# BlockstreamResearch/secp256k1-zkp

Measured on AMD Instinct MI355X. Metric: 64-bit Borromean rangeproof verifies/sec, higher is better.
Workload: dtype u32 limbs (9x29-bit), 32x32->64 integer MAC

## Files before the change

### __graft_entry__.py

```python
import os
import subprocess
import sys

ROOT = os.path.dirname(os.path.abspath(__file__))
CSRC = os.path.join(ROOT, "secp256k1_zkp_amd", "csrc")
HIPCC = os.environ.get("HIPCC", "/opt/rocm/bin/hipcc")
HIP_FLAGS = ["--offload-arch=gfx950", "-O3", "-std=c++17", "-shared", "-fPIC", "-Wno-unused-value"]


def _run(cmd, cwd=None):
    print("+", " ".join(cmd), flush=True)
    subprocess.check_call(cmd, cwd=cwd)


def _stale(target, sources):
    if not os.path.exists(target):
        return True
    t = os.path.getmtime(target)
    return any(os.path.getmtime(s) > t for s in sources if os.path.exists(s))


def build(force=False):
    hdrs = [os.path.join(CSRC, f) for f in os.listdir(CSRC) if f.endswith((".h", ".hip"))] + [os.path.join(ROOT, "include", "secp256k1_zkp_amd.h")]
    sys.path.insert(0, ROOT)
    from secp256k1_zkp_amd import build_lib
    build_lib.build(force=force)
    prims_src = os.path.join(ROOT, "tests", "gpu_prims", "prims.hip")
    prims = os.path.join(ROOT, "tests", "gpu_prims", "libs2k_gpuprims.so")
    if force or _stale(prims, hdrs + [prims_src]):
        _run([HIPCC] + HIP_FLAGS + ["-o", prims, prims_src])
    winv_src = os.path.join(ROOT, "tests", "wave_inverse", "waveinv_test.hip")
    winv = os.path.join(ROOT, "tests", "wave_inverse", "libs2k_waveinv_test.so")
    if force or _stale(winv, hdrs + [winv_src]):
        _run([HIPCC] + HIP_FLAGS + ["-o", winv, winv_src])
    wlanes_src = os.path.join(ROOT, "tests", "wave_inverse", "waveinv_lanes_test.hip")
    wlanes = os.path.join(ROOT, "tests", "wave_inverse", "libs2k_waveinv_lanes_test.so")
    if force or _stale(wlanes, hdrs + [wlanes_src]):
        _run([HIPCC] + HIP_FLAGS + ["-o", wlanes, wlanes_src])
    emu_src = os.path.join(ROOT, "tests", "host_emul", "hostemu.cpp")
    emu = os.path.join(ROOT, "tests", "host_emul", "libs2k_hostemu.so")
    if force or _stale(emu, hdrs + [emu_src]):
        _run(["g++", "-O2", "-std=c++17", "-fPIC", "-shared", "-o", emu, emu_src])
    ecdsa_emu_src = os.path.join(ROOT, "tests", "host_emul", "ecdsa_emu.cpp")
    ecdsa_emu = os.path.join(ROOT, "tests", "host_emul", "libs2k_ecdsa_emu.so")
    if force or _stale(ecdsa_emu, hdrs + [emu_src, ecdsa_emu_src]):
        _run(["g++", "-O2", "-std=c++17", "-fPIC", "-shared", "-o", ecdsa_emu, ecdsa_emu_src])
    wl_emu_src = os.path.join(ROOT, "tests", "host_emul", "whitelist_emu.cpp")
    wl_emu = os.path.join(ROOT, "tests", "host_emul", "libs2k_whitelist_emu.so")
    if force or _stale(wl_emu, hdrs + [emu_src, wl_emu_src]):
        _run(["g++", "-O2", "-std=c++17", "-fPIC", "-shared", "-o", wl_emu, wl_emu_src])
    tw_emu_src = os.path.join(ROOT, "tests", "host_emul", "tweak_emu.cpp")
    tw_emu = os.path.join(ROOT, "tests", "host_emul", "libs2k_tweak_emu.so")
    if force or _stale(tw_emu, hdrs + [emu_src, tw_emu_src]):
        _run(["g++", "-O2", "-std=c++17", "-fPIC", "-shared", "-o", tw_emu, tw_emu_src])
    gen_emu_src = os.path.join(ROOT, "tests", "host_emul", "generator_emu.cpp")
    gen_emu = os.path.join(ROOT, "tests", "host_emul", "libs2k_generator_emu.so")
    if force or _stale(gen_emu, hdrs + [emu_src, gen_emu_src]):
        _run(["g++", "-O2", "-std=c++17", "-fPIC", "-shared", "-o", gen_emu, gen_emu_src])
    ad_emu_src = os.path.join(ROOT, "tests", "host_emul", "adaptor_emu.cpp")
    ad_emu = os.path.join(ROOT, "tests", "host_emul", "libs2k_adaptor_emu.so")
    if force or _stale(ad_emu, hdrs + [emu_src, ad_emu_src]):
        _run(["g++", "-O2", "-std=c++17", "-fPIC", "-shared", "-o", ad_emu, ad_emu_src])
    if os.path.exists(os.path.join(ROOT, "oracle", "zkp_oracle.c")):
        _run(["make", "-s", "-C", os.path.join(ROOT, "oracle"), "oracle"])
    if os.path.isdir(os.environ.get("S2K_REFERENCE", "/root/reference")):
        _run(["make", "-s", "-C", os.path.join(ROOT, "oracle"), "ref", "hooked", "benches", "routed"])
    sys.path.insert(0, ROOT)
    import secp256k1_zkp_amd
    from secp256k1_zkp_amd import _native
    _native.load()


def smoke():
    sys.path.insert(0, ROOT)
    from tests import smoke_impl
    smoke_impl.run()


if __name__ == "__main__":
    build(force="--force" in sys.argv)
    if "--smoke" in sys.argv:
        smoke()
```

### secp256k1_zkp_amd/csrc/ecmult.h

```cpp
#pragma once
#include "group.h"
#include "scalar.h"

#ifndef S2K_GTAB_BITS
#define S2K_GTAB_BITS 26
#endif
#define S2K_GTAB_MAX_BITS 26
#define S2K_GTAB_ENTRY_WORDS 16
#define S2K_GTAB_SWORDS 9
#define S2K_GTAB_MAX_WINDOWS 32
struct gtab_geom { u32 D, W; };
S2K_HD u32 gtab_windows_for(u32 D) { return (256u + D - 1u) / D; }
S2K_HD u32 gtab_top_bits_for(u32 D) { return 256u - D * (gtab_windows_for(D) - 1u); }
S2K_HD int gtab_bits_ok(u32 D) { return D >= 8u && D <= S2K_GTAB_MAX_BITS && gtab_top_bits_for(D) >= 1u && gtab_top_bits_for(D) < D - 1u; }
S2K_HD size_t gtab_slot(u32 D, u32 w, u32 v) { return ((size_t)w << (D - 1u)) + (size_t)v; }
S2K_HD size_t gtab_slots_for(u32 D) { return gtab_slot(D, gtab_windows_for(D), 0) + 1; }
S2K_HD size_t gtab_words_for(u32 D) { return gtab_slots_for(D) * S2K_GTAB_ENTRY_WORDS; }
S2K_HD gtab_geom gtab_geometry(const u32* tab) { gtab_geom g; g.D = tab[0]; g.W = tab[1]; return g; }
S2K_HD void gtab_write_header(u32* tab, u32 D) {
    const u32 W = gtab_windows_for(D);
    tab[0] = D; tab[1] = W;
    for (int i = 0; i < S2K_GTAB_SWORDS; i++) {
        u32 k = 0;
        for (u32 w = 0; w + 1 < W; w++) { const u32 bit = D - 1u + D * w; if ((bit >> 5) == (u32)i) k |= 1u << (bit & 31u); }
        tab[2 + i] = k;
    }
    for (int i = 2 + S2K_GTAB_SWORDS; i < S2K_GTAB_ENTRY_WORDS; i++) tab[i] = 0;
}

S2K_HD void gtab_load(ge& r, const u32* gtab, u32 window, u32 v) {
    const u32* p = gtab + gtab_slot(gtab[0], window, v) * S2K_GTAB_ENTRY_WORDS;
    u32 w[16];
#pragma unroll
    for (int i = 0; i < 16; i++) w[i] = p[i];
    fe_from_words(r.x, w); fe_from_words(r.y, w + 8);
}
S2K_HD void gtab_recode(u32 out[S2K_GTAB_SWORDS], const u32 s[8], const u32* tab) {
    u64 cy = 0;
#pragma unroll
    for (int i = 0; i < S2K_GTAB_SWORDS; i++) {
        cy += (u64)(i < 8 ? s[i] : 0u) + tab[2 + i];
        out[i] = (u32)cy; cy >>= 32;
    }
}
S2K_HD int gtab_locate(const u32*& addr, int& neg, const u32* tab, const gtab_geom& G, int g, u32 lo, u32 hi) {
    const u32 b = (u32)g * G.D;
    const u64 pair = (u64)lo | ((u64)hi << 32);
    const u32 t = (u32)(pair >> (b & 31u)) & ((1u << G.D) - 1u);
    u32 v;
    if ((u32)g + 1u < G.W) { const int d = (int)t - (int)(1u << (G.D - 1u)); neg = d < 0; v = (u32)(d < 0 ? -d : d); }
    else { neg = 0; v = t; }
    if (!v) return 0;
    addr = tab + gtab_slot(G.D, (u32)g, v) * S2K_GTAB_ENTRY_WORDS;
    return 1;
}

#ifndef S2K_PTAB_TWINS
#define S2K_PTAB_TWINS 0
#endif
#define S2K_PTAB_ENTRIES 8
#define S2K_PTAB_ENTRY_WORDS 32
#define S2K_PTAB_TABLE_WORDS (S2K_PTAB_ENTRIES * S2K_PTAB_ENTRY_WORDS)
#define S2K_PTAB_ZISO (2 * S2K_PTAB_TABLE_WORDS)
#define S2K_PTAB_NG (S2K_PTAB_ZISO + 9)
#define S2K_PTAB_WORDS (2 * S2K_PTAB_TABLE_WORDS + 32)

#if defined(__HIP_DEVICE_COMPILE__)
#define S2K_LD_NT(p) __builtin_nontemporal_load(p)
#define S2K_ST_NT(v, p) __builtin_nontemporal_store((v), (p))
#else
#define S2K_LD_NT(p) (*(p))
#define S2K_ST_NT(v, p) (*(p) = (v))
#endif
#ifndef S2K_NT_PARK
#define S2K_NT_PARK 1
#endif
#ifndef S2K_XYZZ_TABLE_PART
#define S2K_XYZZ_TABLE_PART 1
#endif
#ifndef S2K_NT_GTAB_SPLIT
#define S2K_NT_GTAB_SPLIT 0
#endif
#ifndef S2K_NT_GTAB
#define S2K_NT_GTAB 1
#endif
template <int WS = 1>
S2K_HD void ptab_store_raw(u32* e, const fe& x, const fe& y, const fe& third) {
#pragma unroll
    for (int i = 0; i < 9; i++) {
        if (S2K_NT_PARK && WS > 1) { S2K_ST_NT(x.n[i], &e[i * WS]); S2K_ST_NT(y.n[i], &e[(9 + i) * WS]); S2K_ST_NT(third.n[i], &e[(18 + i) * WS]); }
        else { e[i * WS] = x.n[i]; e[(9 + i) * WS] = y.n[i]; e[(18 + i) * WS] = third.n[i]; }
    }
}
template <int N, int WS = 1, int ES = S2K_PTAB_ENTRY_WORDS>
S2K_HD void ptab_build_raw_n(fe& ziso, u32* tab, const gej& A) {
    fe x = A.x, y = A.y; fe_norm_weak(x); fe_norm_weak(y);
    fe zc, s, t, l, nx, s2, qx, qy, w, px, py;
    fe_mul_sqr(zc, y, A.z, s, y);
    fe_neg(nx, x, 1);
    fe_mul_sqr(t, nx, s, l, x);
    fe_mul_int(l, 3); fe_half(l); fe_norm_weak(l);
    fe_sqr2(qx, l, s2, s);
    fe_add(qx, t); fe_add(qx, t); fe_norm_weak(qx);
    fe_add2(w, qx, t);
    fe_mul(qy, l, w); fe_add(qy, s2); fe_neg(qy, qy, 2); fe_norm_weak(qy);
    fe_neg(px, t, 1); py = s2;
    { fe one; fe_set_int(one, 1); ptab_store_raw<WS>(tab, px, py, one); }
    for (int i = 1; i < N; i++) {
        fe dx, dy, c, d, w1, w2, e, a1, x3, y3, tmp;
        fe_neg(dx, px, 4); fe_add(dx, qx); fe_norm_weak(dx);
        fe_neg(dy, py, 3); fe_add(dy, qy); fe_norm_weak(dy);
        fe_sqr2(c, dx, d, dy);
        fe_mul2(w1, qx, c, w2, px, c);
        fe_neg(e, w2, 1); fe_add(e, w1);
        fe_add2(tmp, w1, w2); fe_neg(tmp, tmp, 2);
        fe_add2(x3, d, tmp);
        fe_neg(tmp, x3, 4); fe_add(tmp, w1);
        fe_mul2(a1, qy, e, y3, dy, tmp);
        fe_neg(tmp, a1, 1); fe_add(y3, tmp);
        fe_mul(zc, zc, dx);
        ptab_store_raw<WS>(tab + i * ES, x3, y3, dx);
        px = x3; py = y3; qx = w1; qy = a1;
    }
    ziso = zc;
}
S2K_HD void ptab_build_raw(fe& ziso, u32* tab, const gej& A) { ptab_build_raw_n<S2K_PTAB_ENTRIES>(ziso, tab, A); }
template <int N, int WS = 1, int ES = S2K_PTAB_ENTRY_WORDS>
S2K_HD void ptab_rescale_n(u32* tab, u32* fin, int fin_stride, const fe* zs0) {
    fe zs; if (zs0) zs = *zs0; else fe_set_int(zs, 1);
    u32 nraw[27];
    fe x, y, h;
#pragma unroll
    for (int k = 0; k < 27; k++) nraw[k] = (S2K_NT_PARK && WS > 1) ? S2K_LD_NT(&tab[(N - 1) * ES + k * WS]) : tab[(N - 1) * ES + k * WS];
#pragma unroll
    for (int k = 0; k < 9; k++) { x.n[k] = nraw[k]; y.n[k] = nraw[9 + k]; h.n[k] = nraw[18 + k]; }
    for (int i = N - 1; i >= 0; i--) {
        const u32* er = tab + i * ES;
        u32* e = fin + i * fin_stride;
        if (i > 0) {
#pragma unroll
            for (int k = 0; k < 27; k++) nraw[k] = (S2K_NT_PARK && WS > 1) ? S2K_LD_NT(&er[k * WS - ES]) : er[k * WS - ES];
        }
        if (zs0 || i != N - 1) {
            fe zs2, zs3; fe_sqr(zs2, zs); fe_mul(zs3, zs2, zs);
            fe_mul(x, x, zs2); fe_mul(y, y, zs3);
        }
        fe_normalize(x); fe_normalize(y);
        u32 wx[8], wy[8];
        fe_to_words(wx, x); fe_to_words(wy, y);
#pragma unroll
        for (int k = 0; k < 8; k++) { e[k] = wx[k]; e[8 + k] = wy[k]; }
#if S2K_PTAB_TWINS
        {
            fe beta, bx; fe_set_beta(beta);
            fe_mul(bx, x, beta); fe_normalize(bx);
            u32 wb[8]; fe_to_words(wb, bx);
#pragma unroll
            for (int k = 0; k < 8; k++) { e[16 + k] = wb[k]; e[24 + k] = wy[k]; }
        }
#endif
        fe_mul(zs, zs, h);
        if (i > 0) {
#pragma unroll
            for (int k = 0; k < 27; k++) S2K_CHAIN(nraw[k]);
#pragma unroll
            for (int k = 0; k < 9; k++) { x.n[k] = nraw[k]; y.n[k] = nraw[9 + k]; h.n[k] = nraw[18 + k]; }
        }
    }
}
S2K_HD void ptab_rescale(u32* tab, const fe* zs0) { ptab_rescale_n<S2K_PTAB_ENTRIES>(tab, tab, S2K_PTAB_ENTRY_WORDS, zs0); }
S2K_HD void ptab_build(fe& ziso, u32* ptab, const gej& A) {
    ptab_build_raw(ziso, ptab, A);
    ptab_rescale(ptab, nullptr);
}
S2K_HD void ptab_load_ziso(fe& zi, const u32* ptab) {
#pragma unroll
    for (int i = 0; i < 9; i++) zi.n[i] = ptab[S2K_PTAB_ZISO + i];
}

#if defined(__HIP_DEVICE_COMPILE__)
#define S2K_WAVE_ANY(p) (__any(p))
#define S2K_WAVE_ALL(p) (__all(p))
#define S2K_UNIFORM(x) (__builtin_amdgcn_readfirstlane(x))
#else
#define S2K_WAVE_ANY(p) (p)
#define S2K_WAVE_ALL(p) (p)
#define S2K_UNIFORM(x) (x)
#endif

#define S2K_DIG_WORDS 18
#if defined(__HIP_DEVICE_COMPILE__)
typedef __attribute__((address_space(3))) u32* s2k_lds_ptr;
#define S2K_DIG_STRIDE 256
#define S2K_LANE_DIG(shared_array) ((s2k_lds_ptr)(shared_array) + threadIdx.x)
#else
typedef u32* s2k_lds_ptr;
#define S2K_DIG_STRIDE 1
#define S2K_LANE_DIG(array) (array)
#endif
struct lane_mem { u32* ptab; s2k_lds_ptr dig; };

struct digit_reg { u32 w[5]; };
S2K_HD void digit_reg_init(digit_reg& r, const u32 k[5]) {
    r.w[4] = (k[4] << 31) | (k[3] >> 1);
    r.w[3] = (k[3] << 31) | (k[2] >> 1);
    r.w[2] = (k[2] << 31) | (k[1] >> 1);
    r.w[1] = (k[1] << 31) | (k[0] >> 1);
    r.w[0] = (k[0] << 31);
}
S2K_HD u32 digit_reg_pop(digit_reg& r) {
    const u32 v = r.w[4] >> 28;
#pragma unroll
    for (int i = 4; i > 0; i--) r.w[i] = (r.w[i] << 4) | (r.w[i - 1] >> 28);
    r.w[0] <<= 4;
    return v;
}

#define S2K_ADDS_P 66
#define S2K_ADD_G0 S2K_ADDS_P
#define S2K_ADDS_MAX (S2K_ADD_G0 + S2K_GTAB_MAX_WINDOWS)

S2K_HD void ecmult_lane(gej& R, const gej& A, const scalar& na, const scalar& ng, int has_ng, const u32* gtab, const lane_mem& lm) {
    u32* const ptab = lm.ptab; const s2k_lds_ptr dig = lm.dig;
    S2K_PROF_DECL;
    const int p_active = (!A.inf) & (!sc_is_zero(na));
    const int g_active = has_ng & (!sc_is_zero(ng));
    int hneg0, hneg1;
    fe ziso;
    {
        half_scalar h0, h1;
        sc_split_lambda_odd(h0, h1, na);
        hneg0 = h0.neg; hneg1 = h1.neg;
        {
            digit_reg dr0, dr1; digit_reg_init(dr0, h0.w); digit_reg_init(dr1, h1.w);
            u32 dw[9];
#pragma unroll
            for (int i = 0; i < 9; i++) dw[i] = 0;
#pragma unroll
            for (int i = 2; i < S2K_ADDS_P; i++) { const u32 v = (i & 1) ? digit_reg_pop(dr1) : digit_reg_pop(dr0); dw[i >> 3] |= v << ((i & 7) * 4); }
#pragma unroll
            for (int i = 0; i < 9; i++) dig[i * S2K_DIG_STRIDE] = dw[i];
        }
        S2K_PROF_MARK(1);
        if (S2K_WAVE_ANY(p_active)) {
            ptab_build(ziso, ptab, A);
#pragma unroll
            for (int i = 0; i < 9; i++) ptab[S2K_PTAB_ZISO + i] = ziso.n[i];
        }
    }
    const gtab_geom GG = gtab_geometry(gtab);
    {
        u32 ngr[S2K_GTAB_SWORDS]; gtab_recode(ngr, ng.d, gtab);
#pragma unroll
        for (int i = 0; i < S2K_GTAB_SWORDS; i++) dig[(9 + i) * S2K_DIG_STRIDE] = ngr[i];
    }

    S2K_PROF_MARK(2);
    int a = p_active ? 0 : S2K_ADD_G0;
    int zfixed = !p_active;
    int dbl_left = 0, pending = 0;
    const int a_end = g_active ? S2K_ADD_G0 + (int)GG.W : S2K_ADD_G0;
    auto op_locate = [&](const u32*& addr, int& valid, int& neg, int& lam, int idx) {
        addr = ptab; valid = 0; neg = 0; lam = 0;
        if (idx < S2K_ADD_G0) {
            const int h = idx & 1;
            const int hn = h ? hneg1 : hneg0;
            u32 v = 8u; int flip = hn; valid = 1;
            if (idx >= 2 && idx < S2K_ADDS_P) v = (dig[(idx >> 3) * S2K_DIG_STRIDE] >> ((idx & 7) * 4)) & 15u;
            neg = (v < 8u) ^ flip;
            const u32 e = (v < 8u) ? (7u - v) : (v - 8u);
            addr = ptab + e * S2K_PTAB_ENTRY_WORDS + ((h && S2K_PTAB_TWINS) ? 16 : 0); lam = h && !S2K_PTAB_TWINS;
        } else if (idx < a_end) {
            const int g = idx - S2K_ADD_G0, w = (int)(((u32)g * GG.D) >> 5);
            valid = gtab_locate(addr, neg, gtab, GG, g, dig[(9 + w) * S2K_DIG_STRIDE], w + 1 < S2K_GTAB_SWORDS ? dig[(10 + w) * S2K_DIG_STRIDE] : 0u);
        }
    };
    auto op_decode = [&](ge& o, const u32 raw[16], int neg, int lam) {
        fe y, yn;
        fe_from_words(o.x, raw); fe_from_words(y, raw + 8);
        if (S2K_WAVE_ANY(lam)) {
            fe beta, bx; fe_set_beta(beta); fe_mul(bx, o.x, beta);
            fe_select(o.x, bx, o.x, lam);
        }
        fe_neg(yn, y, 1);
        fe_select(o.y, yn, y, neg);
    };
    const u32* nxt_addr; int nxt_valid, nxt_neg, nxt_lam;
    u32 raw[16];
    ge cur; int cur_valid;
    op_locate(nxt_addr, nxt_valid, nxt_neg, nxt_lam, a);
#pragma unroll
    for (int k = 0; k < 16; k++) raw[k] = nxt_addr[k];
    op_decode(cur, raw, nxt_neg, nxt_lam); cur_valid = nxt_valid;
    gej_set_infinity(R);
    if (p_active) {
        gej_set_ge(R, cur);
        a = 1;
        op_locate(nxt_addr, nxt_valid, nxt_neg, nxt_lam, a);
#pragma unroll
        for (int k = 0; k < 16; k++) raw[k] = nxt_addr[k];
        op_decode(cur, raw, nxt_neg, nxt_lam); cur_valid = nxt_valid;
    }
    op_locate(nxt_addr, nxt_valid, nxt_neg, nxt_lam, a + 1);
#ifndef S2K_NO_FAST_PATH
    if (S2K_WAVE_ALL(p_active) && (S2K_WAVE_ALL(g_active) || !S2K_WAVE_ANY(g_active))) {
        int au = 1;
        while (au < a_end) {
            if (au >= 2 && au < S2K_ADDS_P && !(au & 1)) {
#pragma unroll 1
                for (int k = 0; k < 4; k++) gej_double_lean(R, R);
                S2K_PROF_MARK(6);
            }
            if (au == S2K_ADD_G0) { fe zi; ptab_load_ziso(zi, ptab); fe_mul(R.z, R.z, zi); zfixed = 1; }
#pragma unroll
            for (int k = 0; k < 16; k++) raw[k] = nxt_addr[k];
            gej t; const int same_x = gej_add_ge_lean(t, R, cur);
            if (S2K_WAVE_ANY(same_x & cur_valid)) break;
            if (au < S2K_ADDS_P) R = t;
            else if (cur_valid) R = t;
            au++;
            op_decode(cur, raw, nxt_neg, nxt_lam); cur_valid = nxt_valid;
            op_locate(nxt_addr, nxt_valid, nxt_neg, nxt_lam, au + 1);
        }
        if (au == S2K_ADD_G0 && !zfixed) { fe zi; ptab_load_ziso(zi, ptab); fe_mul(R.z, R.z, zi); zfixed = 1; }
        a = au;
    }
#endif
    int done = !(a < a_end) & zfixed;
    while (S2K_WAVE_ANY(!done)) {
        int do_dbl = 0, do_add = 0;
        if (!done) {
            if (pending) { do_dbl = 1; pending = 0; }
            else if (dbl_left > 0) { do_dbl = !R.inf; dbl_left--; }
            else do_add = 1;
        }
        if (S2K_WAVE_ANY(do_dbl)) {
            gej t; gej_double(t, R);
            if (do_dbl) R = t;
        }
        if (S2K_WAVE_ANY(do_add)) {
#pragma unroll
            for (int k = 0; k < 16; k++) raw[k] = nxt_addr[k];
            gej t; const int f = gej_add_ge(t, R, cur);
            ge nx; op_decode(nx, raw, nxt_neg, nxt_lam);
            if (do_add) {
                if (cur_valid) { R = t; pending = (f == GEJ_ADD_NEEDS_DOUBLE); }
                a++;
                cur = nx; cur_valid = nxt_valid;
                dbl_left = (a >= 2 && a < S2K_ADDS_P && !(a & 1)) ? 4 : 0;
                op_locate(nxt_addr, nxt_valid, nxt_neg, nxt_lam, a + 1);
            }
        }
        const int fix = (!done) & (!zfixed) & (a == S2K_ADD_G0) & (!pending);
        if (S2K_WAVE_ANY(fix)) {
            fe zi;
#pragma unroll
            for (int i = 0; i < 9; i++) zi.n[i] = ptab[S2K_PTAB_ZISO + i];
            fe z; fe_mul(z, R.z, zi);
            if (fix) { R.z = z; zfixed = 1; }
        }
        if ((a >= a_end) & (!pending) & zfixed) done = 1;
    }
    S2K_PROF_MARK(3);
}


#define S2K_SPLIT_ADDS_P 68
struct piece65 { u32 w[3]; int neg; };
S2K_HD void sc_split_pieces(piece65 out[4], const half_scalar& h0, const half_scalar& h1) {
    for (int hf = 0; hf < 2; hf++) {
        const half_scalar& h = hf ? h1 : h0;
        u32 lo[3] = {h.w[0], h.w[1], 0u};
        u32 hi[3] = {h.w[2], h.w[3], h.w[4]};
        int lo_neg = h.neg;
        if (!(hi[0] & 1u)) {
            u32 c = 1u;
            for (int i = 0; i < 3; i++) { const u32 t = hi[i] + c; c = (t < c); hi[i] = t; }
            const u64 l = (u64)lo[0] | ((u64)lo[1] << 32);
            const u64 m = 0ull - l;
            lo[0] = (u32)m; lo[1] = (u32)(m >> 32); lo[2] = 0u;
            lo_neg = !h.neg;
        }
        for (int i = 0; i < 3; i++) { out[hf].w[i] = lo[i]; out[2 + hf].w[i] = hi[i]; }
        out[hf].neg = lo_neg; out[2 + hf].neg = h.neg;
    }
}
S2K_HD int ecmult_lane_split(gej& R, const gej& A, const gej& T, const scalar& na, const scalar& ng, int has_ng, const u32* gtab, const lane_mem& lm) {
    u32* const ptab = lm.ptab; const s2k_lds_ptr dig = lm.dig;
    const int p_active = (!A.inf) & (!T.inf) & (!sc_is_zero(na));
    const int g_active = has_ng & (!sc_is_zero(ng));
    if (!(S2K_WAVE_ALL(p_active) && (S2K_WAVE_ALL(g_active) || !S2K_WAVE_ANY(g_active)))) return 0;
    u32 sneg = 0;
    S2K_PROF_DECL;
    {
        half_scalar h0, h1; sc_split_lambda_odd(h0, h1, na);
        piece65 pc[4]; sc_split_pieces(pc, h0, h1);
        u32 dw[8];
#pragma unroll
        for (int i = 0; i < 8; i++) dw[i] = 0;
#pragma unroll
        for (int st = 0; st < 4; st++) {
            sneg |= (u32)pc[st].neg << st;
#pragma unroll
            for (int pos = 0; pos < 16; pos++) {
                const int i = 15 - pos, bit = 4 * i + 1, word = bit >> 5, sh = bit & 31;
                const u64 pair = (u64)pc[st].w[word] | ((u64)(word + 1 < 3 ? pc[st].w[word + 1] : 0u) << 32);
                const u32 v = (u32)(pair >> sh) & 15u;
                const int nib = pos * 4 + st;
                dw[nib >> 3] |= v << ((nib & 7) * 4);
            }
        }
#pragma unroll
        for (int i = 0; i < 8; i++) dig[i * S2K_DIG_STRIDE] = dw[i];
        {
            u32 ngr[S2K_GTAB_SWORDS]; gtab_recode(ngr, ng.d, gtab);
#pragma unroll
            for (int i = 0; i < S2K_GTAB_SWORDS; i++) dig[(8 + i) * S2K_DIG_STRIDE] = ngr[i];
        }
        fe za, zt, ziso;
        S2K_PROF_MARK(1);
        ptab_build_raw(za, ptab, A);
        ptab_build_raw(zt, ptab + S2K_PTAB_TABLE_WORDS, T);
        S2K_PROF_MARK(8);
        ptab_rescale(ptab, &zt);
        ptab_rescale(ptab + S2K_PTAB_TABLE_WORDS, &za);
        S2K_PROF_MARK(9);
        fe_mul(ziso, za, zt);
#pragma unroll
        for (int i = 0; i < 9; i++) ptab[S2K_PTAB_ZISO + i] = ziso.n[i];
    }
    const gtab_geom GG = gtab_geometry(gtab);
    const int a_g0 = S2K_SPLIT_ADDS_P;
    const int a_end = g_active ? a_g0 + (int)GG.W : a_g0;
    auto op_locate = [&](const u32*& addr, int& valid, int& neg, int& lam, int idx) {
        addr = ptab; valid = 0; neg = 0; lam = 0;
        if (idx < a_g0) {
            const int st = idx & 3;
            u32 v = 8u;
            if (idx >= 4) { const int nib = idx - 4; v = (dig[(nib >> 3) * S2K_DIG_STRIDE] >> ((nib & 7) * 4)) & 15u; }
            valid = 1;
            neg = (v < 8u) ^ (int)((sneg >> st) & 1u);
            const u32 e = (v < 8u) ? (7u - v) : (v - 8u);
            addr = ptab + (st >> 1) * S2K_PTAB_TABLE_WORDS + e * S2K_PTAB_ENTRY_WORDS + (((st & 1) && S2K_PTAB_TWINS) ? 16 : 0); lam = (st & 1) && !S2K_PTAB_TWINS;
        } else if (idx < a_end) {
            const int g = idx - a_g0, w = (int)(((u32)g * GG.D) >> 5);
            valid = gtab_locate(addr, neg, gtab, GG, g, dig[(8 + w) * S2K_DIG_STRIDE], w + 1 < S2K_GTAB_SWORDS ? dig[(9 + w) * S2K_DIG_STRIDE] : 0u);
        }
    };
    auto op_decode = [&](ge& o, const u32 raw[16], int neg, int lam) {
        fe y, yn;
        fe_from_words(o.x, raw); fe_from_words(y, raw + 8);
        if (lam) { fe beta; fe_set_beta(beta); fe_mul(o.x, o.x, beta); }
        fe_neg(yn, y, 1);
        fe_select(o.y, yn, y, neg);
    };
    const u32* nxt_addr; int nxt_valid, nxt_neg, nxt_lam;
    u32 raw[16];
    ge cur; int cur_valid;
    op_locate(nxt_addr, nxt_valid, nxt_neg, nxt_lam, 0);
#pragma unroll
    for (int k = 0; k < 16; k++) raw[k] = nxt_addr[k];
    op_decode(cur, raw, nxt_neg, 0);
    op_locate(nxt_addr, nxt_valid, nxt_neg, nxt_lam, 1);
    int au = 0;
    while (au < a_g0) {
        if (au >= 4 && !(au & 3)) {
#pragma unroll 1
            for (int k = 0; k < 4; k++) gej_double_lean(R, R);
            S2K_PROF_MARK(6);
        }
#pragma unroll
        for (int k = 0; k < 16; k++) raw[k] = nxt_addr[k];
        if (au == 0) gej_set_ge(R, cur);
        else { const int same_x = gej_add_ge_lean(R, R, cur); if (S2K_WAVE_ANY(same_x)) return 0; }
        op_decode(cur, raw, nxt_neg, !S2K_PTAB_TWINS);
        op_locate(nxt_addr, nxt_valid, nxt_neg, nxt_lam, au + 2);
#pragma unroll
        for (int k = 0; k < 16; k++) raw[k] = nxt_addr[k];
        { const int same_x = gej_add_ge_lean(R, R, cur); if (S2K_WAVE_ANY(same_x)) return 0; }
        au += 2;
        op_decode(cur, raw, nxt_neg, 0); cur_valid = nxt_valid;
        op_locate(nxt_addr, nxt_valid, nxt_neg, nxt_lam, au + 1);
    }
    { fe zi; ptab_load_ziso(zi, ptab); fe_mul(R.z, R.z, zi); }
#if S2K_XYZZ_TABLE_PART
    gez acc4; acc4.inf = 0; acc4.x = R.x; acc4.y = R.y;
    fe_sqr(acc4.zz, R.z); fe_mul(acc4.zzz, acc4.zz, R.z);
#endif
    while (au < a_end) {
#if S2K_NT_GTAB_SPLIT && defined(__HIP_DEVICE_COMPILE__)
        {
            typedef unsigned int s2k_u32x4 __attribute__((ext_vector_type(4)));
            const s2k_u32x4* q = (const s2k_u32x4*)nxt_addr;
#pragma unroll
            for (int k = 0; k < 4; k++) { const s2k_u32x4 v = __builtin_nontemporal_load(q + k); raw[4 * k] = v.x; raw[4 * k + 1] = v.y; raw[4 * k + 2] = v.z; raw[4 * k + 3] = v.w; }
        }
#else
#pragma unroll
        for (int k = 0; k < 16; k++) raw[k] = nxt_addr[k];
#endif
#if S2K_XYZZ_TABLE_PART
        {
            gez t = acc4; gez_add_ge_lean(t, cur);
            if (S2K_WAVE_ALL(cur_valid)) acc4 = t;
            else { fe_cmov(acc4.x, t.x, cur_valid); fe_cmov(acc4.y, t.y, cur_valid); fe_cmov(acc4.zz, t.zz, cur_valid); fe_cmov(acc4.zzz, t.zzz, cur_valid); }
        }
#else
        gej t; const int same_x = gej_add_ge_lean(t, R, cur);
        if (S2K_WAVE_ANY(same_x & cur_valid)) return 0;
        if (cur_valid) R = t;
#endif
        au++;
        op_decode(cur, raw, nxt_neg, nxt_lam); cur_valid = nxt_valid;
        op_locate(nxt_addr, nxt_valid, nxt_neg, nxt_lam, au + 1);
    }
#if S2K_XYZZ_TABLE_PART
    if (S2K_WAVE_ANY(fe_normalizes_to_zero(acc4.zz))) return 0;
    gej_set_gez(R, acc4);
#endif
    S2K_PROF_MARK(10);
#ifdef S2K_ON_SPLIT_DONE
    S2K_ON_SPLIT_DONE();
#endif
    return 1;
}


#define S2K_RING_W 5
#define S2K_RING_ENTRIES 16
#define S2K_RING_DIGITS 13
#define S2K_RING_ADDS_P (4 * S2K_RING_DIGITS)
#define S2K_RING_DIG_WORDS 27
#define S2K_RTAB_TABLE_WORDS (S2K_RING_ENTRIES * 16)
#define S2K_RTAB_ZISO (2 * S2K_RTAB_TABLE_WORDS)
#define S2K_RTAB_WORDS (S2K_RTAB_ZISO + 16)
#if defined(__HIP_DEVICE_COMPILE__)
#define S2K_RAW_WS 64
#else
#define S2K_RAW_WS 1
#endif
#define S2K_RAW_ES (27 * S2K_RAW_WS)
#define S2K_RRAW_WAVE_WORDS (2 * S2K_RING_ENTRIES * 27 * 64)

S2K_HD void ecmult_ring_tables(u32* rtab, u32* raw, const gej& C, const gej& T) {
    fe za, zt, ziso;
    u32* const raw_t = raw + S2K_RING_ENTRIES * S2K_RAW_ES;
    ptab_build_raw_n<S2K_RING_ENTRIES, S2K_RAW_WS, S2K_RAW_ES>(za, raw, C);
    ptab_build_raw_n<S2K_RING_ENTRIES, S2K_RAW_WS, S2K_RAW_ES>(zt, raw_t, T);
    ptab_rescale_n<S2K_RING_ENTRIES, S2K_RAW_WS, S2K_RAW_ES>(raw, rtab, 16, &zt);
    ptab_rescale_n<S2K_RING_ENTRIES, S2K_RAW_WS, S2K_RAW_ES>(raw_t, rtab + S2K_RTAB_TABLE_WORDS, 16, &za);
    fe_mul(ziso, za, zt);
#pragma unroll
    for (int i = 0; i < 9; i++) rtab[S2K_RTAB_ZISO + i] = ziso.n[i];
}
S2K_HD int ecmult_ring_step(gej& R, const u32* rtab, const scalar& e, const scalar& s, const scalar& f, int has_f, const u32* gtab, const u32* htab,
                            const s2k_lds_ptr dig) {
    u32 sneg = 0;
    S2K_PROF_DECL;
    {
        half_scalar h0, h1; sc_split_lambda_odd(h0, h1, e);
        piece65 pc[4]; sc_split_pieces(pc, h0, h1);
        u32 dw[9];
#pragma unroll
        for (int i = 0; i < 9; i++) dw[i] = 0;
#pragma unroll
        for (int st = 0; st < 4; st++) {
            sneg |= (u32)pc[st].neg << st;
#pragma unroll
            for (int pos = 0; pos < S2K_RING_DIGITS; pos++) {
                const int i = S2K_RING_DIGITS - 1 - pos, bit = S2K_RING_W * i + 1, word = bit >> 5, sh = bit & 31;
                const u64 pair = (u64)pc[st].w[word] | ((u64)(word + 1 < 3 ? pc[st].w[word + 1] : 0u) << 32);
                u32 v = (u32)(pair >> sh) & 31u;
                if (pos == 0) v |= 16u;
                const int nib = pos * 4 + st;
                dw[nib / 6] |= v << ((nib % 6) * 5);
            }
        }
#pragma unroll
        for (int i = 0; i < 9; i++) dig[i * S2K_DIG_STRIDE] = dw[i];
        u32 sr[S2K_GTAB_SWORDS], fr[S2K_GTAB_SWORDS]; gtab_recode(sr, s.d, gtab); gtab_recode(fr, f.d, has_f ? htab : gtab);
#pragma unroll
        for (int i = 0; i < S2K_GTAB_SWORDS; i++) { dig[(9 + i) * S2K_DIG_STRIDE] = sr[i]; dig[(18 + i) * S2K_DIG_STRIDE] = fr[i]; }
    }
    S2K_PROF_MARK(1);
    const gtab_geom GG = gtab_geometry(gtab), GH = gtab_geometry(has_f ? htab : gtab);
    const int a_g0 = S2K_RING_ADDS_P, a_h0 = a_g0 + (int)GG.W;
    const int a_end = has_f ? a_h0 + (int)GH.W : a_h0;
    auto op_locate = [&](const u32*& addr, int& valid, int& neg, int idx) {
        addr = rtab; valid = 0; neg = 0;
        if (idx < a_g0) {
            const int st = idx & 3;
            const u32 v = (dig[(idx / 6) * S2K_DIG_STRIDE] >> ((idx % 6) * 5)) & 31u;
            valid = 1;
            neg = (v < 16u) ^ (int)((sneg >> st) & 1u);
            const u32 en = (v < 16u) ? (15u - v) : (v - 16u);
            addr = rtab + (st >> 1) * S2K_RTAB_TABLE_WORDS + en * 16;
        } else if (idx < a_end) {
            const int second = idx >= a_h0;
            const int g = idx - (second ? a_h0 : a_g0), base = second ? 18 : 9, w = (int)(((u32)g * (second ? GH.D : GG.D)) >> 5);
            valid = gtab_locate(addr, neg, second ? htab : gtab, second ? GH : GG, g, dig[(base + w) * S2K_DIG_STRIDE], w + 1 < S2K_GTAB_SWORDS ? dig[(base + 1 + w) * S2K_DIG_STRIDE] : 0u);
        }
    };
    auto op_decode = [&](ge& o, const u32 raw[16], int neg, int lam) {
        fe y, yn;
        fe_from_words(o.x, raw); fe_from_words(y, raw + 8);
        if (lam) { fe beta; fe_set_beta(beta); fe_mul(o.x, o.x, beta); }
        fe_neg(yn, y, 1);
        fe_select(o.y, yn, y, neg);
    };
    const u32* nxt_addr; int nxt_valid, nxt_neg;
    u32 raw[16];
    ge cur; int cur_valid;
    op_locate(nxt_addr, nxt_valid, nxt_neg, 0);
#pragma unroll
    for (int k = 0; k < 16; k++) raw[k] = nxt_addr[k];
    op_decode(cur, raw, nxt_neg, 0);
    op_locate(nxt_addr, nxt_valid, nxt_neg, 1);
    int au = 0;
    while (au < a_g0) {
        if (au >= 4 && !(au & 3)) {
            S2K_PROF_MARK(7);
#pragma unroll 1
            for (int k = 0; k < S2K_RING_W; k++) gej_double_lean(R, R);
            S2K_PROF_MARK(6);
        }
#pragma unroll
        for (int k = 0; k < 16; k++) raw[k] = nxt_addr[k];
        if (au == 0) gej_set_ge(R, cur);
        else { const int same_x = gej_add_ge_lean(R, R, cur); if (S2K_WAVE_ANY(same_x)) return 0; }
        op_decode(cur, raw, nxt_neg, 1);
        op_locate(nxt_addr, nxt_valid, nxt_neg, au + 2);
#pragma unroll
        for (int k = 0; k < 16; k++) raw[k] = nxt_addr[k];
        { const int same_x = gej_add_ge_lean(R, R, cur); if (S2K_WAVE_ANY(same_x)) return 0; }
        au += 2;
        op_decode(cur, raw, nxt_neg, 0); cur_valid = nxt_valid;
        op_locate(nxt_addr, nxt_valid, nxt_neg, au + 1);
    }
    S2K_PROF_MARK(7);
    {
        fe zi;
#pragma unroll
        for (int i = 0; i < 9; i++) zi.n[i] = rtab[S2K_RTAB_ZISO + i];
        fe_mul(R.z, R.z, zi);
    }
#if S2K_XYZZ_TABLE_PART
    gez acc4; acc4.inf = 0; acc4.x = R.x; acc4.y = R.y;
    fe_sqr(acc4.zz, R.z); fe_mul(acc4.zzz, acc4.zz, R.z);
#endif
    while (au < a_end) {
#if S2K_NT_GTAB && defined(__HIP_DEVICE_COMPILE__)
        {
            typedef unsigned int s2k_u32x4 __attribute__((ext_vector_type(4)));
            const s2k_u32x4* q = (const s2k_u32x4*)nxt_addr;
#pragma unroll
            for (int k = 0; k < 4; k++) { const s2k_u32x4 v = __builtin_nontemporal_load(q + k); raw[4 * k] = v.x; raw[4 * k + 1] = v.y; raw[4 * k + 2] = v.z; raw[4 * k + 3] = v.w; }
        }
#else
#pragma unroll
        for (int k = 0; k < 16; k++) raw[k] = nxt_addr[k];
#endif
#if S2K_XYZZ_TABLE_PART
        {
            gez t = acc4; gez_add_ge_lean(t, cur);
            if (S2K_WAVE_ALL(cur_valid)) acc4 = t;
            else { fe_cmov(acc4.x, t.x, cur_valid); fe_cmov(acc4.y, t.y, cur_valid); fe_cmov(acc4.zz, t.zz, cur_valid); fe_cmov(acc4.zzz, t.zzz, cur_valid); }
        }
#else
        gej t; const int same_x = gej_add_ge_lean(t, R, cur);
        if (S2K_WAVE_ANY(same_x & cur_valid)) return 0;
        if (cur_valid) R = t;
#endif
        au++;
        op_decode(cur, raw, nxt_neg, 0); cur_valid = nxt_valid;
        op_locate(nxt_addr, nxt_valid, nxt_neg, au + 1);
    }
#if S2K_XYZZ_TABLE_PART
    if (S2K_WAVE_ANY(fe_normalizes_to_zero(acc4.zz))) return 0;
    gej_set_gez(R, acc4);
#endif
    S2K_PROF_MARK(10);
#ifdef S2K_ON_RING_STEP_DONE
    S2K_ON_RING_STEP_DONE();
#endif
    return 1;
}


#define S2K_JOINT_ADDS (4 * 33)
S2K_HD int ecmult_lane2(gej& R, const gej& A, const scalar& na, const gej& B, const scalar& nb, const lane_mem& lm) {
    u32* const ptab = lm.ptab; const s2k_lds_ptr dig = lm.dig;
    const int active = (!A.inf) & (!B.inf) & (!sc_is_zero(na)) & (!sc_is_zero(nb));
    if (!S2K_WAVE_ALL(active)) return 0;
    u32 sneg = 0;
    S2K_PROF_DECL;
    {
        u32 dw[16];
#pragma unroll
        for (int i = 0; i < 16; i++) dw[i] = 0;
        auto put = [&](const half_scalar& h, const int st) {
            sneg |= (u32)h.neg << st;
#pragma unroll
            for (int pos = 0; pos < 32; pos++) {
                const int i = 31 - pos, bit = 4 * i + 1, word = bit >> 5, sh = bit & 31;
                const u64 pair = (u64)h.w[word] | ((u64)h.w[word + 1] << 32);
                const u32 v = (u32)(pair >> sh) & 15u;
                const int nib = pos * 4 + st;
                dw[nib >> 3] |= v << ((nib & 7) * 4);
            }
        };
        { half_scalar h0, h1; sc_split_lambda_odd(h0, h1, na); put(h0, 0); put(h1, 1); }
        { half_scalar h0, h1; sc_split_lambda_odd(h0, h1, nb); put(h0, 2); put(h1, 3); }
#pragma unroll
        for (int i = 0; i < 16; i++) dig[i * S2K_DIG_STRIDE] = dw[i];
        fe za, zb, ziso;
        S2K_PROF_MARK(1);
        ptab_build_raw(za, ptab, A);
        ptab_build_raw(zb, ptab + S2K_PTAB_TABLE_WORDS, B);
        fe_mul(ziso, za, zb);
        if (S2K_WAVE_ANY(fe_normalizes_to_zero(ziso))) return 0;
        S2K_PROF_MARK(8);
        ptab_rescale(ptab, &zb);
        ptab_rescale(ptab + S2K_PTAB_TABLE_WORDS, &za);
        S2K_PROF_MARK(9);
#pragma unroll
        for (int i = 0; i < 9; i++) ptab[S2K_PTAB_ZISO + i] = ziso.n[i];
    }
    auto op_locate = [&](const u32*& addr, int& neg, int idx) {
        const int st = idx & 3;
        u32 v = 8u;
        if (idx >= 4 && idx < S2K_JOINT_ADDS) { const int nib = idx - 4; v = (dig[(nib >> 3) * S2K_DIG_STRIDE] >> ((nib & 7) * 4)) & 15u; }
        neg = (v < 8u) ^ (int)((sneg >> st) & 1u);
        const u32 e = (v < 8u) ? (7u - v) : (v - 8u);
        addr = ptab + (st >> 1) * S2K_PTAB_TABLE_WORDS + e * S2K_PTAB_ENTRY_WORDS + (((st & 1) && S2K_PTAB_TWINS) ? 16 : 0);
    };
    auto op_decode = [&](ge& o, const u32 raw[16], int neg, int lam) {
        fe y, yn;
        fe_from_words(o.x, raw); fe_from_words(y, raw + 8);
        if (lam) { fe beta; fe_set_beta(beta); fe_mul(o.x, o.x, beta); }
        fe_neg(yn, y, 1);
        fe_select(o.y, yn, y, neg);
    };
    const u32* nxt_addr; int nxt_neg;
    u32 raw[16];
    ge cur;
    op_locate(nxt_addr, nxt_neg, 0);
#pragma unroll
    for (int k = 0; k < 16; k++) raw[k] = nxt_addr[k];
    op_decode(cur, raw, nxt_neg, 0);
    op_locate(nxt_addr, nxt_neg, 1);
    int au = 0;
    while (au < S2K_JOINT_ADDS) {
        if (au >= 4 && !(au & 3)) {
#pragma unroll 1
            for (int k = 0; k < 4; k++) gej_double_lean(R, R);
            S2K_PROF_MARK(6);
        }
#pragma unroll
        for (int k = 0; k < 16; k++) raw[k] = nxt_addr[k];
        if (au == 0) gej_set_ge(R, cur);
        else { const int same_x = gej_add_ge_lean(R, R, cur); if (S2K_WAVE_ANY(same_x)) return 0; }
        op_decode(cur, raw, nxt_neg, !S2K_PTAB_TWINS);
        op_locate(nxt_addr, nxt_neg, au + 2);
#pragma unroll
        for (int k = 0; k < 16; k++) raw[k] = nxt_addr[k];
        { const int same_x = gej_add_ge_lean(R, R, cur); if (S2K_WAVE_ANY(same_x)) return 0; }
        au += 2;
        op_decode(cur, raw, nxt_neg, 0);
        op_locate(nxt_addr, nxt_neg, au + 1);
    }
    { fe zi; ptab_load_ziso(zi, ptab); fe_mul(R.z, R.z, zi); }
    S2K_PROF_MARK(10);
#ifdef S2K_ON_JOINT_DONE
    S2K_ON_JOINT_DONE();
#endif
    return 1;
}

#define S2K_PARK_GEJ_WORDS 28
S2K_HD void gej_park(u32* p, size_t stride, const gej& a) {
    fe x = a.x, y = a.y, z = a.z;
    fe_norm_weak(x); fe_norm_weak(y); fe_norm_weak(z);
#pragma unroll
    for (int i = 0; i < 9; i++) { p[i * stride] = x.n[i]; p[(9 + i) * stride] = y.n[i]; p[(18 + i) * stride] = z.n[i]; }
    p[27 * stride] = (u32)a.inf;
}
S2K_HD void gej_unpark(gej& a, const u32* p, size_t stride) {
#pragma unroll
    for (int i = 0; i < 9; i++) { a.x.n[i] = p[i * stride]; a.y.n[i] = p[(9 + i) * stride]; a.z.n[i] = p[(18 + i) * stride]; }
    a.inf = (int)p[27 * stride];
}
template <class Load>
S2K_HD void ecmult_lane2_calls(gej& R, Load load, const u32* gtab, const lane_mem& lm, u32* park, size_t park_stride) {
    scalar zero; sc_set_zero(zero);
    {
        gej P, T; scalar n;
        load(0, P, n);
        ecmult_lane(T, P, n, zero, 0, gtab, lm);
        gej_park(park, park_stride, T);
    }
    gej P, T, F; scalar n;
    load(1, P, n);
    ecmult_lane(T, P, n, zero, 0, gtab, lm);
    gej_unpark(F, park, park_stride);
    gej_add_var(R, F, T);
}
S2K_HD u32 s2k_opaque_zero() { u32 z = 0; S2K_CHAIN(z); return z; }
```

Measured before the change: 1.113 million.

## Use joint C/T combination table for ring multi-scalar step

```diff
diff --git a/__graft_entry__.py b/__graft_entry__.py
--- a/__graft_entry__.py
+++ b/__graft_entry__.py
@@ -61,6 +61,11 @@
     ad_emu = os.path.join(ROOT, "tests", "host_emul", "libs2k_adaptor_emu.so")
     if force or _stale(ad_emu, hdrs + [emu_src, ad_emu_src]):
         _run(["g++", "-O2", "-std=c++17", "-fPIC", "-shared", "-o", ad_emu, ad_emu_src])
+    rj_emu_src = os.path.join(ROOT, "tests", "host_emul", "ring_joint_emu.cpp")
+    for name, flags in (("libs2k_ring_joint_emu.so", []), ("libs2k_ring_joint0_emu.so", ["-DS2K_RING_JOINT=0"])):
+        rj_emu = os.path.join(ROOT, "tests", "host_emul", name)
+        if force or _stale(rj_emu, hdrs + [emu_src, rj_emu_src]):
+            _run(["g++", "-O2", "-std=c++17", "-fPIC", "-shared"] + flags + ["-o", rj_emu, rj_emu_src])
     if os.path.exists(os.path.join(ROOT, "oracle", "zkp_oracle.c")):
         _run(["make", "-s", "-C", os.path.join(ROOT, "oracle"), "oracle"])
     if os.path.isdir(os.environ.get("S2K_REFERENCE", "/root/reference")):
diff --git a/secp256k1_zkp_amd/csrc/ecmult.h b/secp256k1_zkp_amd/csrc/ecmult.h
--- a/secp256k1_zkp_amd/csrc/ecmult.h
+++ b/secp256k1_zkp_amd/csrc/ecmult.h
@@ -526,10 +526,21 @@
 }
 
 
+#ifndef S2K_RING_JOINT
+#define S2K_RING_JOINT 1
+#endif
+#if S2K_RING_JOINT
+#define S2K_RING_W 3
+#define S2K_RING_DIGITS 22
+#define S2K_RING_ADDS_P (2 * S2K_RING_DIGITS)
+#define S2K_RING_GROUP 2
+#else
 #define S2K_RING_W 5
-#define S2K_RING_ENTRIES 16
 #define S2K_RING_DIGITS 13
 #define S2K_RING_ADDS_P (4 * S2K_RING_DIGITS)
+#define S2K_RING_GROUP 4
+#endif
+#define S2K_RING_ENTRIES 16
 #define S2K_RING_DIG_WORDS 27
 #define S2K_RTAB_TABLE_WORDS (S2K_RING_ENTRIES * 16)
 #define S2K_RTAB_ZISO (2 * S2K_RTAB_TABLE_WORDS)
@@ -542,6 +553,123 @@
 #define S2K_RAW_ES (27 * S2K_RAW_WS)
 #define S2K_RRAW_WAVE_WORDS (2 * S2K_RING_ENTRIES * 27 * 64)
 
+#if S2K_RING_JOINT
+S2K_HD void rraw_store(u32* raw, int w, const fe& a) {
+#pragma unroll
+    for (int i = 0; i < 9; i++) {
+        if (S2K_NT_PARK && S2K_RAW_WS > 1) S2K_ST_NT(a.n[i], &raw[(w + i) * S2K_RAW_WS]);
+        else raw[(w + i) * S2K_RAW_WS] = a.n[i];
+    }
+}
+S2K_HD void rraw_load(fe& a, const u32* raw, int w) {
+#pragma unroll
+    for (int i = 0; i < 9; i++) a.n[i] = (S2K_NT_PARK && S2K_RAW_WS > 1) ? S2K_LD_NT(&raw[(w + i) * S2K_RAW_WS]) : raw[(w + i) * S2K_RAW_WS];
+}
+#define S2K_RJ_CHAIN_SLOT 24
+#define S2K_RJ_PAIR0 144
+#define S2K_RJ_PAIR_WORDS 45
+S2K_HD u32 ring_piece_field(const piece65& p, int i) {
+    const int bit = S2K_RING_W * i + 1, word = bit >> 5, sh = bit & 31;
+    const u64 pair = (u64)p.w[word] | ((u64)(word + 1 < 3 ? p.w[word + 1] : 0u) << 32);
+    u32 v = (u32)(pair >> sh) & 7u;
+    if (i == S2K_RING_DIGITS - 1) v |= 4u;
+    return v;
+}
+S2K_HD u32 ring_joint_field(u32 vc, u32 vt, u32 sc, u32 st) {
+    const u32 neg = (u32)(vc < 4u) ^ sc;
+    const u32 ai = vc < 4u ? 3u - vc : vc - 4u;
+    const u32 bi = vt ^ ((neg ^ st) ? 7u : 0u);
+    return (neg << 5) | (ai << 3) | bi;
+}
+S2K_HD void ring_joint_recode(u32 dw[9], const piece65 pc[4]) {
+#pragma unroll
+    for (int i = 0; i < 9; i++) dw[i] = 0;
+#pragma unroll
+    for (int hf = 0; hf < 2; hf++) {
+#pragma unroll
+        for (int pos = 0; pos < S2K_RING_DIGITS; pos++) {
+            const int i = S2K_RING_DIGITS - 1 - pos, idx = pos * 2 + hf;
+            const u32 v = ring_joint_field(ring_piece_field(pc[hf], i), ring_piece_field(pc[2 + hf], i), (u32)pc[hf].neg, (u32)pc[2 + hf].neg);
+            dw[idx / 5] |= v << ((idx % 5) * 6);
+        }
+    }
+}
+S2K_HD void ecmult_ring_tables(u32* rtab, u32* raw, const gej& C, const gej& T) {
+    {
+        fe za, zt, zs;
+        ptab_build_raw_n<4, S2K_RAW_WS, S2K_RAW_ES>(za, raw + S2K_RJ_CHAIN_SLOT * S2K_RAW_ES, C);
+        ptab_build_raw_n<4, S2K_RAW_WS, S2K_RAW_ES>(zt, raw + (S2K_RJ_CHAIN_SLOT + 4) * S2K_RAW_ES, T);
+#pragma unroll 1
+        for (int e = 7; e >= 0; e--) {
+            if ((e & 3) == 3) zs = (e >> 2) ? za : zt;
+            fe x, y, h, zs2, zs3;
+            rraw_load(x, raw, (S2K_RJ_CHAIN_SLOT + e) * 27); rraw_load(y, raw, (S2K_RJ_CHAIN_SLOT + e) * 27 + 9); rraw_load(h, raw, (S2K_RJ_CHAIN_SLOT + e) * 27 + 18);
+            fe_sqr(zs2, zs); fe_mul(zs3, zs2, zs);
+            fe_mul2(x, x, zs2, y, y, zs3);
+            rraw_store(raw, 18 * e, x); rraw_store(raw, 18 * e + 9, y);
+            fe_mul(zs, zs, h);
+        }
+        fe_mul(zs, za, zt);
+#pragma unroll
+        for (int i = 0; i < 9; i++) rtab[S2K_RTAB_ZISO + i] = zs.n[i];
+    }
+    {
+        fe p; fe_set_int(p, 1);
+#pragma unroll 1
+        for (int k = 0; k < 16; k++) {
+            const int w1o = 18 * (k >> 2), w2o = 18 * (4 + (k & 3)), rec = S2K_RJ_PAIR0 + S2K_RJ_PAIR_WORDS * k;
+            fe x1, y1, x2, y2;
+            rraw_load(x1, raw, w1o); rraw_load(y1, raw, w1o + 9); rraw_load(x2, raw, w2o); rraw_load(y2, raw, w2o + 9);
+            fe dx, dy, sy, t, c, d, d2, w1, w2, e, a1, x3, x3m, y3, y3m;
+            fe_neg(t, x1, 1); fe_add2(dx, x2, t); fe_norm_weak(dx);
+            fe_neg(t, y1, 1); fe_add2(dy, y2, t); fe_norm_weak(dy);
+            fe_add2(sy, y1, y2); fe_norm_weak(sy);
+            fe_sqr2(c, dx, d, dy);
+            fe_mul2(w1, x1, c, w2, x2, c);
+            fe_neg(e, w1, 1); fe_add(e, w2);
+            fe_mul_sqr(a1, y1, e, d2, sy);
+            fe_add2(t, w1, w2); fe_neg(t, t, 2);
+            fe_add2(x3, d, t); fe_add2(x3m, d2, t);
+            fe_neg(t, x3, 4); fe_add(t, w1);
+            fe_neg(e, w1, 1); fe_add(e, x3m);
+            fe_mul2(y3, dy, t, y3m, sy, e);
+            fe_neg(t, a1, 1); fe_add(y3, t); fe_add(y3m, t);
+            rraw_store(raw, rec, x3); rraw_store(raw, rec + 9, y3); rraw_store(raw, rec + 18, x3m); rraw_store(raw, rec + 27, y3m);
+            rraw_store(raw, rec + 36, p);
+            fe_mul(p, p, dx);
+        }
+    }
+    fe s; fe_set_int(s, 1);
+#pragma unroll 1
+    for (int k = 15; k >= 0; k--) {
+        const int ai = k >> 2, bi = k & 3, rec = S2K_RJ_PAIR0 + S2K_RJ_PAIR_WORDS * k;
+        fe xp, yp, xm, ym, m, x1, dx;
+        rraw_load(xp, raw, rec); rraw_load(yp, raw, rec + 9); rraw_load(xm, raw, rec + 18); rraw_load(ym, raw, rec + 27); rraw_load(m, raw, rec + 36);
+        rraw_load(x1, raw, 18 * ai); rraw_load(dx, raw, 18 * (4 + bi));
+        fe_neg(x1, x1, 1); fe_add(dx, x1); fe_norm_weak(dx);
+        fe_mul2(m, m, s, s, s, dx);
+        fe m2, m3; fe_sqr(m2, m); fe_mul(m3, m2, m);
+        fe_mul2(xp, xp, m2, xm, xm, m2);
+        fe_mul2(yp, yp, m3, ym, ym, m3);
+        fe_normalize(xp); fe_normalize(yp); fe_normalize(xm); fe_normalize(ym);
+        u32* const ep = rtab + (ai * 8 + 4 + bi) * 16;
+        u32* const em = rtab + (ai * 8 + 3 - bi) * 16;
+        u32 wx[8], wy[8];
+        fe_to_words(wx, xp); fe_to_words(wy, yp);
+#pragma unroll
+        for (int i = 0; i < 8; i++) { ep[i] = wx[i]; ep[8 + i] = wy[i]; }
+        fe_to_words(wx, xm); fe_to_words(wy, ym);
+#pragma unroll
+        for (int i = 0; i < 8; i++) { em[i] = wx[i]; em[8 + i] = wy[i]; }
+    }
+    fe ziso;
+#pragma unroll
+    for (int i = 0; i < 9; i++) ziso.n[i] = rtab[S2K_RTAB_ZISO + i];
+    fe_mul(ziso, ziso, s);
+#pragma unroll
+    for (int i = 0; i < 9; i++) rtab[S2K_RTAB_ZISO + i] = ziso.n[i];
+}
+#else
 S2K_HD void ecmult_ring_tables(u32* rtab, u32* raw, const gej& C, const gej& T) {
     fe za, zt, ziso;
     u32* const raw_t = raw + S2K_RING_ENTRIES * S2K_RAW_ES;
@@ -553,14 +681,20 @@
 #pragma unroll
     for (int i = 0; i < 9; i++) rtab[S2K_RTAB_ZISO + i] = ziso.n[i];
 }
+#endif
 S2K_HD int ecmult_ring_step(gej& R, const u32* rtab, const scalar& e, const scalar& s, const scalar& f, int has_f, const u32* gtab, const u32* htab,
                             const s2k_lds_ptr dig) {
+#if !S2K_RING_JOINT
     u32 sneg = 0;
+#endif
     S2K_PROF_DECL;
     {
         half_scalar h0, h1; sc_split_lambda_odd(h0, h1, e);
         piece65 pc[4]; sc_split_pieces(pc, h0, h1);
         u32 dw[9];
+#if S2K_RING_JOINT
+        ring_joint_recode(dw, pc);
+#else
 #pragma unroll
         for (int i = 0; i < 9; i++) dw[i] = 0;
 #pragma unroll
@@ -576,6 +710,7 @@
                 dw[nib / 6] |= v << ((nib % 6) * 5);
             }
         }
+#endif
 #pragma unroll
         for (int i = 0; i < 9; i++) dig[i * S2K_DIG_STRIDE] = dw[i];
         u32 sr[S2K_GTAB_SWORDS], fr[S2K_GTAB_SWORDS]; gtab_recode(sr, s.d, gtab); gtab_recode(fr, f.d, has_f ? htab : gtab);
@@ -589,12 +724,19 @@
     auto op_locate = [&](const u32*& addr, int& valid, int& neg, int idx) {
         addr = rtab; valid = 0; neg = 0;
         if (idx < a_g0) {
+#if S2K_RING_JOINT
+            const u32 v = (dig[(idx / 5) * S2K_DIG_STRIDE] >> ((idx % 5) * 6)) & 63u;
+            valid = 1;
+            neg = (int)(v >> 5);
+            addr = rtab + (v & 31u) * 16;
+#else
             const int st = idx & 3;
             const u32 v = (dig[(idx / 6) * S2K_DIG_STRIDE] >> ((idx % 6) * 5)) & 31u;
             valid = 1;
             neg = (v < 16u) ^ (int)((sneg >> st) & 1u);
             const u32 en = (v < 16u) ? (15u - v) : (v - 16u);
             addr = rtab + (st >> 1) * S2K_RTAB_TABLE_WORDS + en * 16;
+#endif
         } else if (idx < a_end) {
             const int second = idx >= a_h0;
             const int g = idx - (second ? a_h0 : a_g0), base = second ? 18 : 9, w = (int)(((u32)g * (second ? GH.D : GG.D)) >> 5);
@@ -618,7 +760,7 @@
     op_locate(nxt_addr, nxt_valid, nxt_neg, 1);
     int au = 0;
     while (au < a_g0) {
-        if (au >= 4 && !(au & 3)) {
+        if (au >= S2K_RING_GROUP && !(au & (S2K_RING_GROUP - 1))) {
             S2K_PROF_MARK(7);
 #pragma unroll 1
             for (int k = 0; k < S2K_RING_W; k++) gej_double_lean(R, R);
@@ -643,6 +785,9 @@
 #pragma unroll
         for (int i = 0; i < 9; i++) zi.n[i] = rtab[S2K_RTAB_ZISO + i];
         fe_mul(R.z, R.z, zi);
+#if S2K_RING_JOINT && !S2K_XYZZ_TABLE_PART
+        if (S2K_WAVE_ANY(fe_normalizes_to_zero(zi))) return 0;
+#endif
     }
 #if S2K_XYZZ_TABLE_PART
     gez acc4; acc4.inf = 0; acc4.x = R.x; acc4.y = R.y;
```

After: 1.144 million, median of 6. 1.03x the previous value.
